# ACCtools/alignasm

Hardware: AMD Instinct MI355X
Metric: contigs_per_sec (higher is better)
Workload: dtype int64

## Files before the change

### alignasm_amd/csrc/aasm_gpu.hip

```cpp
#include <hip/hip_runtime.h>
#include <initializer_list>

#include <atomic>
#include <chrono>
#include <mutex>
#include <thread>
#include <fcntl.h>
#include <sys/mman.h>
#include <sys/stat.h>
#include <unistd.h>

#include "aasm_pipeline.h"
#include "aasm_ksw.h"
#include "aasm_cut.h"
#include "aasm_read.h"
#include "aasm_paf.hpp"

namespace aasm {

__device__ inline int64_t xcd_bid(int64_t b, int64_t g, int on) {
    if (!on || g < 64) return b;
    const int64_t g8 = g & ~(int64_t)7;
    return b < g8 ? (b & 7) * (g8 >> 3) + (b >> 3) : b;
}
// ... 177 lines not shown
        int64_t oa = sh_carry[0], ob = sh_carry[1], ta = 0, tb = 0;
#pragma unroll
        for (int i = 0; i < 16; i++) { const int64_t xa = sh_w[0][i], xb = sh_w[1][i]; if (i < wv) { oa += xa; ob += xb; } ta += xa; tb += xb; }
        int64_t ra = oa + ia - sa, rb = ob + ib - sb;
#pragma unroll
        for (int i = 0; i < 4; i++) { if (i0 + i < n) { out_a[i0 + i] = ra; if (in_b) out_b[i0 + i] = rb; } ra += va[i]; rb += vb[i]; }
        __syncthreads();
        if (threadIdx.x == 0) { sh_carry[0] += ta; sh_carry[1] += tb; }
        __syncthreads();
    }
    if (threadIdx.x == 0) { out_a[n] = sh_carry[0]; if (in_b) out_b[n] = sh_carry[1]; }
}

struct ScalarSrc { const int64_t *p[12]; };
__global__ void aasm_read_scalars(ScalarSrc src, int n, int64_t *dst) {
    const int i = (int)threadIdx.x;
    if (i < n) __hip_atomic_store(dst + i, *src.p[i], __ATOMIC_RELAXED, __HIP_MEMORY_SCOPE_SYSTEM);
}

struct ArenaBlock { char *p; size_t cap, used; };

struct DevCtx {
    int device = -1;
    bool ready = false;
    hipStream_t stream = nullptr, side = nullptr, side2 = nullptr;
    hipEvent_t ev_fork, ev_join, ev_fork2, ev_join2, ev_fork_b;
    int64_t *d_scratch2 = nullptr;
    size_t d_scratch2_cap = 0;
    std::vector<ArenaBlock> blocks;
    int64_t *pinned = nullptr;
    int64_t *pinned_dev = nullptr;
    char *stage[2] = {nullptr, nullptr};
    int64_t *d_scratch = nullptr;
    size_t d_scratch_cap = 0;
    uint64_t generation = 0;
    std::atomic<int> input_arrived{0};
    std::mutex mu;
    hipEvent_t ev_b[AASM_N_PHASES], ev_e[AASM_N_PHASES], ev_t0, ev_t1;
    int n_events_made = 0;
    int n_events2 = 0;
    hipEvent_t *timing_event(int i) { return i < AASM_N_PHASES ? &ev_b[i] : i < 2 * AASM_N_PHASES ? &ev_e[i - AASM_N_PHASES] : i == 2 * AASM_N_PHASES ? &ev_t0 : &ev_t1; }
    bool events = false;
    size_t peak_bytes = 0;
    std::vector<hipEvent_t> export_events;
};

static void drain_exports(DevCtx &cx) {
    for (hipEvent_t e : cx.export_events) { (void)hipEventSynchronize(e); (void)hipEventDestroy(e); }
    cx.export_events.clear();
}
static DevCtx g_ctx[16];
static std::mutex g_init_mu;
static std::atomic<int64_t> g_n_range_splits{0}, g_n_device_mallocs{0}, g_n_stream_syncs{0}, g_n_read_slow_rows{0}, g_n_read_fallbacks{0};

static std::string hip_err(const char *what, hipError_t e) {
    return std::string(what) + ": " + hipGetErrorString(e);
}

static int ctx_init(int device) {
    if (device < 0 || device >= 16) { set_last_error("device ordinal out of range"); return AASM_E_INVAL; }
    std::lock_guard<std::mutex> lk(g_init_mu);
    DevCtx &cx = g_ctx[device];
    if (cx.ready) return AASM_OK;
    int n = 0;
    hipError_t e = hipGetDeviceCount(&n);
    if (e != hipSuccess || n <= 0) { set_last_error("no HIP device available (this library has no CPU fallback)"); return AASM_E_NODEVICE; }
    if (device >= n) { set_last_error("device ordinal beyond hipGetDeviceCount"); return AASM_E_NODEVICE; }
    if ((e = hipSetDevice(device)) != hipSuccess) { set_last_error(hip_err("hipSetDevice", e)); return AASM_E_NODEVICE; }
    auto fail = [&](const char *what, hipError_t err) {
        set_last_error(hip_err(what, err));
        if (cx.pinned) { hipHostFree(cx.pinned); cx.pinned = nullptr; }
        if (cx.n_events_made > 0) { hipEventDestroy(cx.ev_fork); }
        if (cx.n_events_made > 1) { hipEventDestroy(cx.ev_join); }
        for (int i = 2; i < cx.n_events_made; i++) hipEventDestroy(*cx.timing_event(i - 2));
        cx.n_events_made = 0;
        if (cx.n_events2 > 0) { hipEventDestroy(cx.ev_fork2); }
        if (cx.n_events2 > 1) { hipEventDestroy(cx.ev_join2); }
        if (cx.n_events2 > 2) { hipEventDestroy(cx.ev_fork_b); }
        cx.n_events2 = 0;
        if (cx.side2) { hipStreamDestroy(cx.side2); cx.side2 = nullptr; }
        if (cx.side) { hipStreamDestroy(cx.side); cx.side = nullptr; }
        if (cx.stream) { hipStreamDestroy(cx.stream); cx.stream = nullptr; }
        return AASM_E_NODEVICE;
    };
    if ((e = hipStreamCreateWithFlags(&cx.stream, hipStreamNonBlocking)) != hipSuccess) return fail("hipStreamCreate", e);
    if ((e = hipStreamCreateWithFlags(&cx.side, hipStreamNonBlocking)) != hipSuccess) return fail("hipStreamCreate", e);
    if ((e = hipStreamCreateWithFlags(&cx.side2, hipStreamNonBlocking)) != hipSuccess) return fail("hipStreamCreate", e);
    if ((e = hipEventCreateWithFlags(&cx.ev_fork2, hipEventDisableTiming)) != hipSuccess) return fail("hipEventCreate", e);
    cx.n_events2 = 1;
    if ((e = hipEventCreateWithFlags(&cx.ev_join2, hipEventDisableTiming)) != hipSuccess) return fail("hipEventCreate", e);
    cx.n_events2 = 2;
    if ((e = hipEventCreateWithFlags(&cx.ev_fork_b, hipEventDisableTiming)) != hipSuccess) return fail("hipEventCreate", e);
    cx.n_events2 = 3;
    if ((e = hipEventCreateWithFlags(&cx.ev_fork, hipEventDisableTiming)) != hipSuccess) return fail("hipEventCreate", e);
    cx.n_events_made = 1;
    if ((e = hipEventCreateWithFlags(&cx.ev_join, hipEventDisableTiming)) != hipSuccess) return fail("hipEventCreate", e);
    cx.n_events_made = 2;
    for (int i = 0; i < 2 * AASM_N_PHASES + 2; i++) {
        if ((e = hipEventCreate(cx.timing_event(i))) != hipSuccess) return fail("hipEventCreate", e);
        cx.n_events_made++;
    }
    if ((e = hipHostMalloc((void **)&cx.pinned, 64 * sizeof(int64_t), hipHostMallocMapped)) != hipSuccess) return fail("hipHostMalloc", e);
    std::memset(cx.pinned, 0, 64 * sizeof(int64_t));
    if ((e = hipHostGetDevicePointer((void **)&cx.pinned_dev, cx.pinned, 0)) != hipSuccess) return fail("hipHostGetDevicePointer", e);
    cx.events = true;
    cx.device = device;
// ... 275 lines not shown

static thread_local int64_t g_bad_record = -1;

static int solve_on_device(DevCtx &cx, const aasm_batch_in &dev_in, const aasm_opts &opts, hipStream_t stream, aasm_result **res_out,
                           GpuBackend **be_out) {
    GpuBackend *be = *be_out;
    const bool timing = opts.collect_timing != 0;
    aasm_result *res = new aasm_result();
    res->device = cx.device; res->stream = stream;
    std::memset(&res->stats, 0, sizeof(res->stats));
    if (timing) hipEventRecord(cx.ev_t0, stream);
    be->test_dirty_scan = decode_hooks(opts).dirty_scan;
    int rc = run_pipeline(*be, dev_in, opts, res->w, res->sz);
    if (rc == AASM_OK) rc = pack_alloc(*be, res->w, res->pk);
    be->flush_zero();
    if (timing) hipEventRecord(cx.ev_t1, stream);
    be->join();
    be->join2();
    hipError_t e = hipStreamSynchronize(stream);
    if (e == hipSuccess) e = hipStreamSynchronize(cx.side);
    if (e == hipSuccess) e = hipStreamSynchronize(cx.side2);
    be->scan_stalled();
    if (rc == AASM_OK && be->failed()) rc = be->oom() ? AASM_E_NOMEM : AASM_E_HIP;
    if (rc == AASM_OK && e != hipSuccess) { set_last_error(hip_err("pipeline", e)); rc = AASM_E_HIP; }
    if (rc == AASM_E_PARSE) {
        g_bad_record = res->sz.bad_record;
        set_last_error("malformed cs:Z tag in record " + std::to_string(res->sz.bad_record) + " of the batch");
    }
    if (rc == AASM_E_HIP || rc == AASM_E_NOMEM || be->failed() || cx.pinned[SCAN_STALL_SLOT] != 0) {
        (void)hipDeviceSynchronize();
        if (cx.d_scratch) (void)hipMemset(cx.d_scratch, 0, cx.d_scratch_cap * 8);
        if (cx.d_scratch2) (void)hipMemset(cx.d_scratch2, 0, cx.d_scratch2_cap * 8);
        cx.pinned[SCAN_STALL_SLOT] = 0;
        (void)hipGetLastError();
    }
    if (rc != AASM_OK) { delete res; return rc; }
    if (timing) {
        for (int i = 0; i < AASM_N_PHASES; i++)
            if (be->phase_used[i]) { float ms = 0; if (hipEventElapsedTime(&ms, cx.ev_b[i], cx.ev_e[i]) == hipSuccess) res->stats.phase_ms[i] = ms; }
        float ms = 0;
        if (hipEventElapsedTime(&ms, cx.ev_t0, cx.ev_t1) == hipSuccess) res->stats.total_ms = ms;
    }
    {
        int64_t cnt[CNT_N];
        std::memset(cnt, 0, sizeof(cnt));
        be->d2h(cnt, res->w.counters, sizeof(cnt));
        aasm_stats &st = res->stats;
        st.n_vertices = res->sz.VT; st.n_edges = res->sz.ET;
        st.n_pairs = res->sz.S > 0 ? be->read_i64(res->w.ov_rank + res->sz.S) : 0;
        st.n_heap_nodes = cnt[CNT_HEAPNODES]; st.n_paths_found = cnt[CNT_PATHS]; st.n_paths_converted = cnt[CNT_CONVERTED];
        st.n_unconnectable = cnt[CNT_UNCONN]; st.range_steps = cnt[CNT_RANGE_STEPS];
        st.ispr_edges = cnt[CNT_ISPR_E]; st.ispr_vertices = cnt[CNT_ISPR_V]; st.path_edges = cnt[CNT_PATH_E];
        st.out_elems = cnt[CNT_OUT_E]; st.pq_pushes = cnt[CNT_PQ_PUSH];
        if (be->failed()) { delete res; return AASM_E_HIP; }
    }
    res->stats.device_bytes = (int64_t)be->bytes;
    res->generation = cx.generation;
    res->named = be->named;
    *res_out = res;
    return AASM_OK;
}

extern "C" {

int aasm_abi_version(void) { return AASM_ABI_VERSION; }

int aasm_device_count(void) {
    int n = 0;
    if (hipGetDeviceCount(&n) != hipSuccess) return 0;
    return n;
}

int aasm_init(int device) { return ctx_init(device); }

int aasm_solve_device(const aasm_batch_in *dev_in, const aasm_opts *opts, void *stream, aasm_result **res) {
    if (!dev_in || !res) return AASM_E_INVAL;
    aasm_opts o;
    std::memset(&o, 0, sizeof(o));
    if (opts) o = *opts;
    int rc = ctx_init(o.device);
    if (rc != AASM_OK) return rc;
    DevCtx &cx = g_ctx[o.device];
    std::lock_guard<std::mutex> lk(cx.mu);
    hipSetDevice(o.device);
    hipStream_t s = stream ? (hipStream_t)stream : cx.stream;
    GpuBackend be(cx, s, o.collect_timing != 0);
    GpuBackend *bp = &be;
    return solve_on_device(cx, *dev_in, o, s, res, &bp);
}

int aasm_result_stats(const aasm_result *res, aasm_stats *stats) {
    if (!res || !stats) return AASM_E_INVAL;
    *stats = res->stats;
    return AASM_OK;
}

namespace {
#define AASM_STAGE_BYTES ((size_t)16 << 20)
struct FetchBackend {
    DevCtx &cx; hipStream_t stream; bool fail = false;
    void d2h(void *dst, const void *src, size_t n) {
        if (fail || n == 0) return;
        hipError_t e = hipMemcpyAsync(dst, src, n, hipMemcpyDeviceToHost, stream);
        if (e == hipSuccess) e = hipStreamSynchronize(stream);
        if (e != hipSuccess) { set_last_error(hip_err("hipMemcpy D2H", e)); fail = true; }
    }
// ... 191 lines not shown
    std::vector<int32_t> ones((size_t)n_contigs, 1);
    w.dupflag = (int32_t *)m.up(ones.data(), (size_t)n_contigs * 4);
#if defined(AASM_KPROF)
    w.prof_heap = (int64_t *)filled((size_t)n_contigs * 64, 0);
#endif
    if (!m.ok) return be.err();
    launch_kernel(KN_SORT_FIX, n_contigs, kern_block[KN_SORT_FIX], be.stream, w);
    if (!be.launched() || !be.d2h(perm_out, w.perm, (size_t)R * 4)) return be.err();
#if defined(AASM_KPROF)
    {
        std::vector<int64_t> kp((size_t)n_contigs * 8);
        be.d2h(kp.data(), w.prof_heap, kp.size() * 8);
        double mean[8] = {0};
        for (int64_t c = 0; c < n_contigs; c++) for (int i = 0; i < 8; i++) mean[i] += (double)kp[(size_t)c * 8 + i] / (double)n_contigs;
        fprintf(stderr, "sort_fix sections (mean cycles): load %.0f  A %.0f  B %.0f  C %.0f  global partitions %.0f  wave lifetime %.1f us\n", mean[0], mean[1], mean[2], mean[3], mean[4], mean[7] / 100.0);
    }
#endif
    return AASM_OK;
}

int aasm_sssp_dijkstra(int64_t n_graphs, const int64_t *g_voff, const int64_t *rowptr, const int32_t *col, const int64_t *w5,
                       const int32_t *src, int64_t *d5, int32_t *prev, int device) {
    const char *why = "";
    const int rc = dijkstra_check_args(n_graphs, g_voff, rowptr, col, w5, src, d5, prev, &why);
    return graph_entry("aasm_sssp_dijkstra", rc, why, device, [&](GraphGpu &be) { return dijkstra_run(be, n_graphs, g_voff, rowptr, col, w5, src, d5, prev, &why); });
}

int aasm_sssp_dial(int64_t n_graphs, const int64_t *g_voff, const int64_t *rowptr, const int32_t *col, const int32_t *cost,
                   const int32_t *src, int lim, int64_t *dist, int64_t *pre, int device) {
    const char *why = "";
    const int rc = dial_check_args(n_graphs, g_voff, rowptr, col, cost, src, lim, dist, pre, &why);
    return graph_entry("aasm_sssp_dial", rc, why, device, [&](GraphGpu &be) { return dial_run(be, n_graphs, g_voff, rowptr, col, cost, src, lim, dist, pre, &why); });
}

int aasm_k_shortest_walks(int64_t n_graphs, const int64_t *g_voff, const int64_t *rowptr, const int32_t *col, const int64_t *w5,
                          const int32_t *source, const int32_t *sink, int64_t k, int flags, int device, aasm_ksw_out *out) {
    const char *why = "";
    const int rc = ksw_check_args(n_graphs, g_voff, rowptr, col, w5, source, sink, k, flags, out, &why);
    return graph_entry("aasm_k_shortest_walks", rc, why, device, [&](GraphGpu &be) {
        return ksw_run(be, n_graphs, g_voff, rowptr, col, w5, source, sink, k, flags, out, (int64_t)4 << 30);
    });
}

void aasm_ksw_free(aasm_ksw_out *out) { ksw_free_out(out); }

int64_t aasm_debug_counter(const char *name) {
    if (!name) return -1;
    const std::string n(name);
    if (n == "range_splits") return g_n_range_splits.load();
    if (n == "device_mallocs") return g_n_device_mallocs.load();
    if (n == "stream_syncs") return g_n_stream_syncs.load();
    if (n == "read_slow_rows") return g_n_read_slow_rows.load();
    if (n == "read_host_fallbacks") return g_n_read_fallbacks.load();
    return -1;
}

int64_t aasm_debug_fetch(aasm_result *res, const char *name, void *dst, int64_t dst_bytes) {
    if (!res || !name) return AASM_E_INVAL;
    DevCtx &cx = g_ctx[res->device];
    std::lock_guard<std::mutex> lk(cx.mu);
    if (res->generation != cx.generation) return AASM_E_INVAL;
    auto it = res->named.find(name);
    if (it == res->named.end()) return AASM_E_INVAL;
    if (dst) {
        hipSetDevice(res->device);
        size_t n = std::min<size_t>((size_t)dst_bytes, it->second.second);
        hipError_t e = hipMemcpy(dst, it->second.first, n, hipMemcpyDeviceToHost);
        if (e != hipSuccess) { set_last_error(hip_err("debug fetch", e)); return AASM_E_HIP; }
    }
    return (int64_t)it->second.second;
}

struct aasm_upload { int device; std::vector<void *> ptrs; aasm_batch_in view; };

static int upload_range(const aasm_batch_in *in, int64_t c0, int64_t c1, int device, aasm_upload **up_out, aasm_batch_in *dev_view) {
    if (!in || !up_out || !dev_view || c0 < 0 || c1 > in->n_contigs || c0 >= c1) return AASM_E_INVAL;
    int rc = ctx_init(device);
    if (rc != AASM_OK) return rc;
    hipSetDevice(device);
    g_ctx[device].input_arrived.store(1);
    aasm_upload *up = new aasm_upload();
    up->device = device;
    bool ok = true, oom = false;
    std::string why = "the batch carries neither match ranges nor cs tags";
    auto put = [&](const void *src, size_t bytes) -> void * {
        void *p = nullptr;
        if (!ok) return nullptr;
        hipError_t e = hipMalloc(&p, bytes ? bytes : 8);
        if (e != hipSuccess) { ok = false; oom = (e == hipErrorOutOfMemory); (void)hipGetLastError(); why = hip_err("hipMalloc(upload)", e); return nullptr; }
        up->ptrs.push_back(p);
        if (bytes && (e = hipMemcpy(p, src, bytes, hipMemcpyHostToDevice)) != hipSuccess) { ok = false; why = hip_err("hipMemcpy H2D", e); }
        return p;
    };
    const int64_t C = c1 - c0, r0 = in->ctg_rec_off[c0], r1 = in->ctg_rec_off[c1], R = r1 - r0;
    const int64_t g0 = in->rec_rng_off[r0], g1 = in->rec_rng_off[r1], G = g1 - g0;
    std::vector<int64_t> coff(C + 1), roff(R + 1);
    for (int64_t c = 0; c <= C; c++) coff[c] = in->ctg_rec_off[c0 + c] - r0;
    for (int64_t r = 0; r <= R; r++) roff[r] = in->rec_rng_off[r0 + r] - g0;
    aasm_batch_in &v = up->view;
    v.n_contigs = C; v.n_records = R; v.n_ranges = G;
    v.ctg_rec_off = (const int64_t *)put(coff.data(), (C + 1) * 8);
    v.qry_str = (const int64_t *)put(in->qry_str + r0, R * 8);
    v.qry_end = (const int64_t *)put(in->qry_end + r0, R * 8);
    v.ref_str = (const int64_t *)put(in->ref_str + r0, R * 8);
    v.ref_end = (const int64_t *)put(in->ref_end + r0, R * 8);
    v.qry_total = (const int64_t *)put(in->qry_total + r0, R * 8);
// ... 406 lines not shown
```

### alignasm_amd/csrc/aasm_kernels.h

```cpp
#pragma once
#include <cstddef>
#include "aasm_dev.h"
#include "../../include/alignasm_amd.h"

namespace aasm {

struct PqK;
struct WS {
    int64_t C, R, R0, S, VT, ET;
    int32_t K, nsl;
    int32_t avg_sidetracks;
    int32_t xcd_map;
    int32_t mw_compact;
    int32_t sort_depth_test;
    const int64_t *rec_off, *in_qs, *in_qe, *in_rs, *in_re, *in_qt, *in_rng_off, *rql, *rqr, *rrl;
    const int32_t *in_chr;
    const uint8_t *in_fwd, *in_mq;
    const char *cs_text;
    const int64_t *cs_off;
    int64_t *rng_rec;
    int64_t rng_stride;
    int32_t *cs_bad;
    int32_t *perm, *dupflag, *np, *pstart;
    int64_t *s_qs, *s_qe, *s_rs, *s_re, *s_qt, *s_rb;
// ... 24 lines not shown
    I4 *kcand;
    PqK *pq;
    int64_t pq_stride;
    int32_t *pathA, *pathB, *pathT, *pre2, *stamp;
    Dist *dist2;
    uint8_t *notalt;
    int32_t *mark_time;
    int32_t *plan_kk;
    int32_t *nconv, *cv_ctg, *cv_k, *cv_ord, *cv_kind, *cv_szr, *cv_szv, *cv_n, *cv_err, *cv_path, *cv_pre2, *cv_stamp, *cv_la;
    int64_t *conv_off, *cv_roff, *cv_voff, *cv_cov;
    OutElem *cv_out;
    Dist *cv_dist2;
    int64_t NCONV;
    OutElem *cur_out, *main_out, *alt_out, *pool;
    int32_t *main_len, *alt_len, *all_gen, *all_seq;
    int32_t *ar_ctg, *ar_gen, *ar_seq, *ar_len;
    int64_t *ar_off;
    int64_t pool_cap, ar_cap;
    int64_t *main_off, *alt_off;
    OutElem *main_c, *alt_c;
    int32_t *status;
    int64_t *counters;
    int32_t *gb_flag; int32_t gb_off;
    int64_t *prof_heap, *prof_sel, *prof_gb;
    Dist *st_cost;
    int32_t *st_n;
    I4 *vhdr, *vhdr2, *cinfo;
    int32_t mw_mode;
    int32_t *mw_flag, *mw_lg;
    HNode *hprov;
    int64_t *mw_off;
    int32_t *mw_cap;
    int32_t *mw_order, *mw_rs, *mw_fb;
    int32_t *mw_rsv, *mw_used;
    int32_t *mw_list, *mw_sorted;
    int32_t *mw_key;
    int32_t mw_n, mw_base;
    I4 *tnx;
    int32_t *tnx16;
    I4 *rvh;
    I4 *r_pk;
    I4 *fvh;
    int32_t chain_mode;
    int32_t chain_all, chain_minN;
    int32_t chain_test;
    int32_t *chain_flag, *chain_list;
    int32_t *pend;
    int32_t *cq;
    I4 *bfsq;
    int32_t chain_ord;
    int32_t chain_rn;
};

enum { CNT_RANGE_STEPS = 0, CNT_UNCONN, CNT_POOL, CNT_AR, CNT_CONVERTED, CNT_HEAPNODES, CNT_PATHS, CNT_OVF, CNT_ISPR_E, CNT_ISPR_V, CNT_PATH_E, CNT_OUT_E, CNT_PQ_PUSH, CNT_MW, CNT_MAXN, CNT_LONGSORT, CNT_MAXV, CNT_CHAIN, CNT_GB_S, CNT_GB_L, CNT_GB_REST, CNT_N };

AASM_DEV void set_status(const WS &w, int64_t c, int code) { if (w.status[c] == 0) w.status[c] = code; }
AASM_DEV bool in_chain_class(const WS &w, int64_t c) { return w.chain_flag != nullptr && w.chain_flag[c] != 0; }
AASM_DEV bool in_graph_class(const WS &w, int64_t c) { return w.gb_flag && w.gb_flag[c] != 0; }
#define AASM_COORD_LIMIT ((int64_t)1 << 40)
AASM_DEV bool coord_ok(int64_t x) { return x >= 0 && x < AASM_COORD_LIMIT; }

struct CsScan {
    int64_t q, rr, val, n, cnt, o0;
    int32_t plen;
    int t;
    bool fwd, bad;
};
AASM_DEV void cs_close_op(CsScan &s, const WS &w) {
    if (s.t == ':') {
        if (s.plen < 1 || s.val <= 0 || s.n >= s.cnt) { s.bad = true; return; }
        if (s.fwd) {
            const int64_t o = s.o0 + s.n;
            I4 lo, hi; const int64_t qr = s.q + s.val - 1;
            lo.x = lo32((uint64_t)s.q); lo.y = hi32((uint64_t)s.q); lo.z = lo32((uint64_t)qr); lo.w = hi32((uint64_t)qr);
            hi.x = lo32((uint64_t)s.rr); hi.y = hi32((uint64_t)s.rr); hi.z = 0; hi.w = 0;
            I4 *rec = (I4 *)(w.rng_rec + 4 * o); rec[0] = lo; rec[1] = hi;
            s.q += s.val;
        } else {
            const int64_t o = s.o0 + s.cnt - 1 - s.n;
            I4 lo, hi; const int64_t ql = s.q - s.val, qr = s.q - 1, rl = s.rr + s.val - 1;
            lo.x = lo32((uint64_t)ql); lo.y = hi32((uint64_t)ql); lo.z = lo32((uint64_t)qr); lo.w = hi32((uint64_t)qr);
            hi.x = lo32((uint64_t)rl); hi.y = hi32((uint64_t)rl); hi.z = 0; hi.w = 0;
            I4 *rec = (I4 *)(w.rng_rec + 4 * o); rec[0] = lo; rec[1] = hi;
            s.q -= s.val;
        }
        s.rr += s.val;
        s.n++;
    } else if (s.t == '*') {
        if (s.plen != 2) { s.bad = true; return; }
        s.q += s.fwd ? 1 : -1; s.rr += 1;
    } else {
        if (s.plen < 1) { s.bad = true; return; }
        if (s.t == '+') s.q += s.fwd ? s.plen : -s.plen; else s.rr += s.plen;
    }
}
AASM_DEV void kb_cs_ranges(const KCtx &k, const WS &w) {
    const int64_t br = k.bid * k.nthreads + k.tid;
    if (br >= w.R) return;
    const int64_t r = w.R0 + br;
    const int64_t p0 = w.cs_off[r], len = w.cs_off[r + 1] - p0;
    const uint8_t *cs = (const uint8_t *)w.cs_text + p0;
    const int64_t qs = w.in_qs[r], qe = w.in_qe[r], rs = w.in_rs[r], re = w.in_re[r];
    CsScan s;
    s.fwd = w.in_fwd[r] != 0;
    s.o0 = w.in_rng_off[r]; s.cnt = w.in_rng_off[r + 1] - s.o0;
    s.q = s.fwd ? qs : qe + 1; s.rr = s.fwd ? rs : re;
    s.val = 0; s.n = 0; s.plen = 0; s.t = 0;
// ... 1367 lines not shown
        for (int i = 0; i < GB_U; i++) {
            const int64_t e = eb + (en[i] & 0xffffu);
            const bool in = p0 + i * nth < E;
            hv[i] = in ? w.e_col[e] : 0; wq[i] = in ? w.e_wq[e] : 0; wr[i] = in ? w.e_wr[e] : 0; fl[i] = in ? w.e_fl[e] : 0;
        }
        AASM_UNROLL
        for (int i = 0; i < GB_U; i++) {
            if (p0 + i * nth >= E) break;
            const uint32_t key = en[i] & 0xffffu;
            const I4 rec = pack_in_edge((int32_t)(en[i] >> 16), wq[i], wr[i], fl[i]);
            const int32_t l0 = L->rp[hv[i]], l1 = L->rp[hv[i] + 1];
            int32_t rank = 0, j = l0;
            for (; j + 4 <= l1; j += 4) {
                const uint32_t k0 = L->ks[j], k1 = L->ks[j + 1], k2 = L->ks[j + 2], k3 = L->ks[j + 3];
                rank += (k0 < key) + (k1 < key) + (k2 < key) + (k3 < key);
            }
            for (; j < l1; j++) rank += (L->ks[j] < key) ? 1 : 0;
            w.r_pk[eb + l0 + rank] = rec;
            if (rank < 2) w.rvh[3 * (vb + hv[i]) + 1 + rank] = rec;
        }
    }
    KPROF_STAMP(3);
    for (int32_t v0 = tid; v0 < V; v0 += GB_U * nth) {
        int64_t o0[GB_U], o1[GB_U];
        I4 f1[GB_U];
        AASM_UNROLL
        for (int i = 0; i < GB_U; i++) { const int32_t v = v0 + i * nth; const bool in = v < V; o0[i] = in ? w.rowptr[vb + v] : 0; o1[i] = in ? w.rowptr[vb + v + 1] : 0; }
        AASM_UNROLL
        for (int i = 0; i < GB_U; i++) f1[i] = fwd_hdr_heads(w, o0[i], o1[i]);
        AASM_UNROLL
        for (int i = 0; i < GB_U; i++) {
            const int32_t v = v0 + i * nth;
            if (v >= V) break;
            const int64_t gv = vb + v;
            const int32_t ideg = L->rp[v + 1] - L->rp[v];
            const int64_t r0 = eb + L->rp[v];
            I4 h, z;
            z.x = z.y = z.z = z.w = 0;
            h.x = (int32_t)(uint32_t)(uint64_t)r0; h.y = (int32_t)((uint64_t)r0 >> 32); h.z = ideg; h.w = 0;
            w.rptr[gv] = r0;
            w.rvh[3 * gv] = h;
            if (ideg < 1) w.rvh[3 * gv + 1] = z;
            if (ideg < 2) w.rvh[3 * gv + 2] = z;
            sweep_vertex_store(w, gv, ideg, o0[i], o1[i], f1[i], vb + V);
        }
    }
    KPROF_STAMP(4);
    KPROF_FLUSH(w.prof_gb, c, tid);
}

#ifndef AASM_SWEEP_G
#define AASM_SWEEP_G (AASM_WAVE >= 32 ? 32 : 1)
#endif
template <int G> struct SweepGrp {
    static constexpr int N = AASM_WAVE / G;
    int g, gl;
    AASM_MEM explicit SweepGrp(int lane) : g(lane / G), gl(lane % G) {}
    AASM_MEM uint32_t bits(uint64_t m) const { return G >= 64 ? 0u : (uint32_t)((m >> (g * (G & 63))) & ((1ull << (G & 63)) - 1ull)); }
    AASM_MEM int32_t below(uint64_t m) const {
        if (G >= 64) return popc64(m & lanemask_lt(gl));
        return __builtin_popcount(bits(m) & ((1u << gl) - 1u));
    }
    AASM_MEM int32_t count(uint64_t m) const { return G >= 64 ? popc64(m) : __builtin_popcount(bits(m)); }
};

struct ChainSync { int32_t tail_pub, sweep_done, prep_done, ord_pub, ord_done, pad[3]; };
#if defined(AASM_HOST_EMUL)
AASM_DEV void st_shared_i32(int32_t *p, int32_t v) { *p = v; }
#else
AASM_DEV void st_shared_i32(int32_t *p, int32_t v) { __hip_atomic_store(p, v, __ATOMIC_RELAXED, __HIP_MEMORY_SCOPE_WORKGROUP); }
#endif

template <int G, bool PUB = false>
AASM_DEV void kb_rev_sweep(const KCtx &k, const WS &w, ChainSync *S = nullptr) {
    const SweepGrp<G> sg(k.lane);
    const int64_t c = k.bid * SweepGrp<G>::N + sg.g;
    const bool valid = c < w.C && (PUB || !in_chain_class(w, c));
    const int64_t V = valid ? (int64_t)w.ctgV[c] : 0;
    const int64_t vb = valid ? w.voff[c] : 0;
    RevQ *Q = (RevQ *)k.lds + sg.g;
    Dist *d = w.sp_d + vb;
    int32_t *best = w.sp_best + vb, *q = w.rev_order + vb, *cnt = w.cnt_tmp + vb;
    const I4 *rvh = w.rvh + 3 * vb;
    int32_t tail = 0, lds_hi = 0;
    for (int64_t base = 0; wave_any(base < V); base += G) {
        const int64_t v = base + sg.gl;
        const bool z = v < V && cnt[v] == 0;
        const uint64_t m = wave_ballot(z);
        const int32_t at = tail + sg.below(m);
        if (z) {
            q[at] = (int32_t)v;
            if (at < REVQ_N) { RevEnt *E = &Q->e[at]; I4 hd = rvh[3 * v]; hd.w = (int32_t)v; E->hdr = hd; E->d = d[v]; E->rec[0] = rvh[3 * v + 1]; E->rec[1] = rvh[3 * v + 2]; }
        }
        tail += sg.count(m);
    }
    lds_hi = tail < REVQ_N ? tail : REVQ_N;
    wave_lds_sync();
    int32_t pub = 0;
    if (PUB) { pub = uni(tail); store_drain(); st_shared_i32(&S->tail_pub, pub); }
    int32_t head = 0;
    while (wave_any(head < tail)) {
        const bool live = head < tail;
        RevEnt *E = &Q->e[head & (REVQ_N - 1)];
        if (wave_any(live && head >= lds_hi)) {
            if (live && head >= lds_hi && sg.gl == 0) { const int32_t v = q[head]; I4 hd = rvh[3 * v]; hd.w = v; E->hdr = hd; E->d = d[v]; E->rec[0] = rvh[3 * v + 1]; E->rec[1] = rvh[3 * v + 2]; }
            wave_lds_sync();
        }
        I4 hd; hd.x = hd.y = hd.z = hd.w = 0;
        Dist dv = dist_max();
        if (live) { hd = E->hdr; dv = E->d; head++; }
        const int32_t deg = hd.z, v = hd.w;
        const int64_t r0 = (int64_t)(((uint64_t)(uint32_t)hd.y << 32) | (uint32_t)hd.x);
        const bool reach = dv.anom >= 0;
        for (int32_t base = 0; wave_any(base < deg); base += G) {
            const int32_t t = base + sg.gl;
            const bool act = t < deg;
            bool z = false;
            int32_t u = 0;
            I4 uh0, uh1, uh2;
            Dist du = dist_max();
            uh0.x = uh0.y = uh0.z = uh0.w = 0; uh1 = uh0; uh2 = uh0;
            if (act) {
                I4 rc;
                if (t < 2) rc = E->rec[t];
                else { rc = w.r_pk[r0 + t]; asm volatile("" ::: "memory"); }
                u = rc.x;
                Dist wd;
                wd.qry = (int64_t)(((uint64_t)(uint32_t)rc.z << 32) | (uint32_t)rc.y); wd.ref = rc.w & 0xffffff;
                const int32_t fl = (int32_t)((uint32_t)rc.w >> 24);
                wd.anom = fl & 3; wd.qnz = (fl >> 2) & 1; wd.qtot = (fl >> 3) & 1; wd.pad = 0;
                du = d[u];
                const int32_t left = cnt[u] - 1;
                uh0 = rvh[3 * u]; uh1 = rvh[3 * u + 1]; uh2 = rvh[3 * u + 2];
                const Dist cand = dist_add(dv, wd);
                const int64_t sc = cand.qry + cand.ref, su = du.qry + du.ref;
                const int32_t tc = cand.qtot ? cand.qtot : 1, tu = du.qtot ? du.qtot : 1;
                const bool better = reach & ((du.anom < 0) | (sc < su) | ((sc == su) & ((cand.anom < du.anom) | ((cand.anom == du.anom) & ((int64_t)cand.qnz * tu > (int64_t)du.qnz * tc)))));
                if (better) { du = cand; d[u] = cand; best[u] = v; }
                cnt[u] = left;
                z = left == 0;
            }
            const uint64_t m = wave_ballot(z);
            const int32_t at = tail + sg.below(m);
            if (z) {
                q[at] = u;
                if (lds_hi == tail && at - head < REVQ_N - 1) { RevEnt *N = &Q->e[at & (REVQ_N - 1)]; uh0.w = u; N->hdr = uh0; N->d = du; N->rec[0] = uh1; N->rec[1] = uh2; }
            }
            const int32_t nnew = sg.count(m);
            if (lds_hi == tail) { int32_t room = REVQ_N - 1 - (tail - head); if (room > nnew) room = nnew; if (room < 0) room = 0; lds_hi += room; }
            tail += nnew;
        }
        wave_lds_sync();
        if (PUB) {
            const int32_t tu = uni(tail);
            if (tu != pub) { store_drain(); st_shared_i32(&S->tail_pub, tu); pub = tu; }
        }
    }
    if (valid && tail != (int32_t)V && sg.gl == 0) set_status(w, c, -6);
    if (PUB) { store_drain(); st_shared_i32(&S->sweep_done, 1); }
}

struct FwdEnt { I4 a, b; };
struct FwdQ { FwdEnt e[REVQ_N]; };
#define AASM_FWD_LDS_BYTES (REVQ_N * 32)
static_assert(sizeof(FwdQ) <= AASM_FWD_LDS_BYTES, "LDS budget");
template <int G>
AASM_DEV void kb_fwd_sweep(const KCtx &k, const WS &w) {
    const SweepGrp<G> sg(k.lane);
    const int64_t c = k.bid * SweepGrp<G>::N + sg.g;
    const bool valid = c < w.C;
    const int64_t V = valid ? (int64_t)w.ctgV[c] : 0;
    const int64_t vb = valid ? w.voff[c] : 0;
    FwdQ *Q = (FwdQ *)k.lds + sg.g;
    int32_t *q = w.fwd_order + vb, *pos = w.fwd_pos + vb, *cnt = w.cnt_tmp2 + vb, *an = w.an + vb;
    const I4 *fvh = w.fvh + 2 * vb;
    int32_t tail = 0, lds_hi = 0;
    for (int64_t base = 0; wave_any(base < V); base += G) {
        const int64_t v = base + sg.gl;
        const bool z = v < V && cnt[v] == 0;
        const uint64_t m = wave_ballot(z);
        if (z) {
            const int32_t t = tail + sg.below(m);
            q[t] = (int32_t)v; pos[v] = t;
            if (t < REVQ_N) { I4 fa = fvh[2 * v], fb = fvh[2 * v + 1]; fa.w = (int32_t)v; fb.x = an[v]; Q->e[t].a = fa; Q->e[t].b = fb; }
        }
        tail += sg.count(m);
    }
    lds_hi = tail < REVQ_N ? tail : REVQ_N;
    wave_lds_sync();
    int32_t head = 0;
    while (wave_any(head < tail)) {
        const bool live = head < tail;
        FwdEnt *E = &Q->e[head & (REVQ_N - 1)];
        if (wave_any(live && head >= lds_hi)) {
            if (live && head >= lds_hi && sg.gl == 0) { const int32_t u = q[head]; I4 fa = fvh[2 * u], fb = fvh[2 * u + 1]; fa.w = u; fb.x = an[u]; E->a = fa; E->b = fb; }
            wave_lds_sync();
        }
        I4 fa, fb; fa.x = fa.y = fa.z = fa.w = 0; fb = fa;
        if (live) { fa = E->a; fb = E->b; head++; }
        const int32_t deg = fa.z, au = fb.x;
        const int64_t r0 = (int64_t)(((uint64_t)(uint32_t)fa.y << 32) | (uint32_t)fa.x);
        for (int32_t base = 0; wave_any(base < deg); base += G) {
            const int32_t t = base + sg.gl;
            const bool act = t < deg;
            bool z = false;
            int32_t v = 0, av = -1;
            I4 va, vbb;
            va.x = va.y = va.z = va.w = 0; vbb = va;
            if (act) {
                int32_t wa;
                if (t < 2) { v = t == 0 ? fb.y : fb.z; wa = (fb.w >> (8 * t)) & 3; }
                else { v = w.e_col[r0 + t]; wa = w.e_fl[r0 + t] & 3; }
                av = an[v];
                const int32_t left = cnt[v] - 1;
                va = fvh[2 * v]; vbb = fvh[2 * v + 1];
                const int32_t nd = au + wa;
                if ((au >= 0) & ((av < 0) | (nd < av))) { av = nd; an[v] = nd; }
                cnt[v] = left;
                z = left == 0;
            }
            const uint64_t m = wave_ballot(z);
            const int32_t at = tail + sg.below(m);
            if (z) {
                q[at] = v; pos[v] = at;
                if (lds_hi == tail && at - head < REVQ_N - 1) { FwdEnt *N = &Q->e[at & (REVQ_N - 1)]; va.w = v; vbb.x = av; N->a = va; N->b = vbb; }
            }
            const int32_t nnew = sg.count(m);
            if (lds_hi == tail) { int32_t room = REVQ_N - 1 - (tail - head); if (room > nnew) room = nnew; if (room < 0) room = 0; lds_hi += room; }
            tail += nnew;
        }
        wave_lds_sync();
    }
    if (valid && sg.gl == 0 && V > 0) {
        w.anom_dest[c] = an[V - 1];
        if (tail != (int32_t)V) set_status(w, c, -6);
    }
}

AASM_DEV void kb_topo_count(const KCtx &k, const WS &w) {
    const int64_t gp = k.bid * k.nthreads + k.tid;
    if (gp >= w.VT) return;
    const int64_t vb = w.voff[w.v_ctg[gp]];
    const int32_t u = w.fwd_order[gp];
    w.tp_deg[gp] = (int32_t)(w.rowptr[vb + u + 1] - w.rowptr[vb + u]);
    w.tp_vj[gp] = w.v_j[vb + u];
}
AASM_DEV void kb_topo_fill(const KCtx &k, const WS &w) {
    const int64_t gp = k.bid * AASM_WAVE + k.lane;
    const bool act = gp < w.VT;
    int64_t vb = 0, r0 = 0, t0 = 0;
    int32_t deg = 0;
    if (act) {
        vb = w.voff[w.v_ctg[gp]];
        const int32_t u = w.fwd_order[gp];
        r0 = w.rowptr[vb + u]; deg = w.tp_deg[gp]; t0 = w.tp_ptr[gp];
    }
    const bool big = deg > AASM_LONG_ROW;
    if (act && !big)
        for (int32_t t = 0; t < deg; t++) {
            w.te_pk[t0 + t] = pack_in_edge(w.fwd_pos[vb + w.e_col[r0 + t]], w.e_wq[r0 + t], w.e_wr[r0 + t], w.e_fl[r0 + t]);
        }
    uint64_t bigmask = wave_ballot(big);
    while (bigmask) {
        const int src = ffs64(bigmask) - 1;
        bigmask &= bigmask - 1;
        const int64_t vb2 = wave_bcast(vb, src), r02 = wave_bcast(r0, src), t02 = wave_bcast(t0, src);
        const int32_t deg2 = wave_bcast(deg, src);
        for (int32_t t = k.lane; t < deg2; t += AASM_WAVE) {
            w.te_pk[t02 + t] = pack_in_edge(w.fwd_pos[vb2 + w.e_col[r02 + t]], w.e_wq[r02 + t], w.e_wr[r02 + t], w.e_fl[r02 + t]);
        }
    }
}

AASM_DEV int32_t children_vertex(const WS &w, int64_t gv, int32_t *ch4 = nullptr) {
    const int64_t vb = w.voff[w.v_ctg[gv]];
    const int32_t u = (int32_t)(gv - vb);
    const int64_t r0 = w.rptr[gv], r1 = w.rptr[gv + 1];
    int32_t n = 0, prev = -1;
    int32_t c0 = -1, c1 = -1, c2 = -1, c3 = -1;
    for (int64_t t = r0; t < r1; t += 4) {
        int32_t src[4], bst[4];
        AASM_UNROLL
        for (int i = 0; i < 4; i++) src[i] = (t + i < r1) ? w.r_pk[t + i].x : -1;
        AASM_UNROLL
        for (int i = 0; i < 4; i++) bst[i] = src[i] >= 0 ? w.sp_best[vb + src[i]] : -1;
// ... 2302 lines not shown
```

Baseline: 445,800.

## Process two queue vertices per iteration in reverse and forward topo sweeps

Both the reverse and the forward topological sweep kernels now consume two queued vertices per loop iteration when one has low degree. Their edges are packed into the same subgroup lanes, which cuts the number of serial wave iterations and LDS syncs on chain-like graphs. Conflicts where the second vertex depends on the first are found with ballots: the reverse sweep falls back to a single vertex, and the forward sweep folds the dependent update into one lane. New counters track how many pairs are formed. This adds branch complexity and register pressure, and any error in the dependency handling could change the results.

```diff
diff --git a/alignasm_amd/csrc/aasm_gpu.hip b/alignasm_amd/csrc/aasm_gpu.hip
--- a/alignasm_amd/csrc/aasm_gpu.hip
+++ b/alignasm_amd/csrc/aasm_gpu.hip
@@ -253,6 +253,7 @@
 static DevCtx g_ctx[16];
 static std::mutex g_init_mu;
 static std::atomic<int64_t> g_n_range_splits{0}, g_n_device_mallocs{0}, g_n_stream_syncs{0}, g_n_read_slow_rows{0}, g_n_read_fallbacks{0};
+static std::atomic<int64_t> g_n_sweep_pairs_rev{0}, g_n_sweep_pairs_fwd{0};
 
 static std::string hip_err(const char *what, hipError_t e) {
     return std::string(what) + ": " + hipGetErrorString(e);
@@ -634,6 +635,7 @@
         st.n_unconnectable = cnt[CNT_UNCONN]; st.range_steps = cnt[CNT_RANGE_STEPS];
         st.ispr_edges = cnt[CNT_ISPR_E]; st.ispr_vertices = cnt[CNT_ISPR_V]; st.path_edges = cnt[CNT_PATH_E];
         st.out_elems = cnt[CNT_OUT_E]; st.pq_pushes = cnt[CNT_PQ_PUSH];
+        g_n_sweep_pairs_rev += cnt[CNT_PAIR_REV]; g_n_sweep_pairs_fwd += cnt[CNT_PAIR_FWD];
         if (be->failed()) { delete res; return AASM_E_HIP; }
     }
     res->stats.device_bytes = (int64_t)be->bytes;
@@ -931,6 +933,8 @@
     if (n == "stream_syncs") return g_n_stream_syncs.load();
     if (n == "read_slow_rows") return g_n_read_slow_rows.load();
     if (n == "read_host_fallbacks") return g_n_read_fallbacks.load();
+    if (n == "sweep_pairs_rev") return g_n_sweep_pairs_rev.load();
+    if (n == "sweep_pairs_fwd") return g_n_sweep_pairs_fwd.load();
     return -1;
 }
 
diff --git a/alignasm_amd/csrc/aasm_kernels.h b/alignasm_amd/csrc/aasm_kernels.h
--- a/alignasm_amd/csrc/aasm_kernels.h
+++ b/alignasm_amd/csrc/aasm_kernels.h
@@ -100,7 +100,7 @@
     int32_t chain_rn;
 };
 
-enum { CNT_RANGE_STEPS = 0, CNT_UNCONN, CNT_POOL, CNT_AR, CNT_CONVERTED, CNT_HEAPNODES, CNT_PATHS, CNT_OVF, CNT_ISPR_E, CNT_ISPR_V, CNT_PATH_E, CNT_OUT_E, CNT_PQ_PUSH, CNT_MW, CNT_MAXN, CNT_LONGSORT, CNT_MAXV, CNT_CHAIN, CNT_GB_S, CNT_GB_L, CNT_GB_REST, CNT_N };
+enum { CNT_RANGE_STEPS = 0, CNT_UNCONN, CNT_POOL, CNT_AR, CNT_CONVERTED, CNT_HEAPNODES, CNT_PATHS, CNT_OVF, CNT_ISPR_E, CNT_ISPR_V, CNT_PATH_E, CNT_OUT_E, CNT_PQ_PUSH, CNT_MW, CNT_MAXN, CNT_LONGSORT, CNT_MAXV, CNT_CHAIN, CNT_GB_S, CNT_GB_L, CNT_GB_REST, CNT_PAIR_REV, CNT_PAIR_FWD, CNT_N };
 
 AASM_DEV void set_status(const WS &w, int64_t c, int code) { if (w.status[c] == 0) w.status[c] = code; }
 AASM_DEV bool in_chain_class(const WS &w, int64_t c) { return w.chain_flag != nullptr && w.chain_flag[c] != 0; }
@@ -1574,6 +1574,15 @@
 #ifndef AASM_SWEEP_G
 #define AASM_SWEEP_G (AASM_WAVE >= 32 ? 32 : 1)
 #endif
+#ifndef AASM_SWEEP_PAIR
+#define AASM_SWEEP_PAIR 1
+#endif
+#ifndef AASM_SWEEP_PAIR_REV
+#define AASM_SWEEP_PAIR_REV AASM_SWEEP_PAIR
+#endif
+#ifndef AASM_SWEEP_PAIR_FWD
+#define AASM_SWEEP_PAIR_FWD AASM_SWEEP_PAIR
+#endif
 template <int G> struct SweepGrp {
     static constexpr int N = AASM_WAVE / G;
     int g, gl;
@@ -1584,6 +1593,7 @@
         return __builtin_popcount(bits(m) & ((1u << gl) - 1u));
     }
     AASM_MEM int32_t count(uint64_t m) const { return G >= 64 ? popc64(m) : __builtin_popcount(bits(m)); }
+    AASM_MEM bool any(uint64_t m) const { return G >= 64 ? m != 0 : bits(m) != 0u; }
 };
 
 struct ChainSync { int32_t tail_pub, sweep_done, prep_done, ord_pub, ord_done, pad[3]; };
@@ -1620,7 +1630,8 @@
     wave_lds_sync();
     int32_t pub = 0;
     if (PUB) { pub = uni(tail); store_drain(); st_shared_i32(&S->tail_pub, pub); }
-    int32_t head = 0;
+    constexpr bool PAIR = AASM_SWEEP_PAIR_REV != 0 && G > 1;
+    int32_t head = 0, npair = 0;
     while (wave_any(head < tail)) {
         const bool live = head < tail;
         RevEnt *E = &Q->e[head & (REVQ_N - 1)];
@@ -1628,6 +1639,69 @@
             if (live && head >= lds_hi && sg.gl == 0) { const int32_t v = q[head]; I4 hd = rvh[3 * v]; hd.w = v; E->hdr = hd; E->d = d[v]; E->rec[0] = rvh[3 * v + 1]; E->rec[1] = rvh[3 * v + 2]; }
             wave_lds_sync();
         }
+        if constexpr (PAIR) {
+        RevEnt *E1 = &Q->e[(head + 1) & (REVQ_N - 1)];
+        bool pair = live && head + 1 < lds_hi;
+        int32_t deg0 = 0, deg1 = 0;
+        if (live) deg0 = E->hdr.z;
+        if (pair) deg1 = E1->hdr.z;
+        pair = pair && (deg0 <= 2 || deg1 <= 2);
+        if (!pair) deg1 = 0;
+        for (int32_t base = 0; wave_any(base < deg0 + deg1); base += G) {
+            const int32_t t = base + sg.gl;
+            const bool e1 = t >= deg0;
+            const int32_t te = e1 ? t - deg0 : t;
+            bool act = t < deg0 + deg1;
+            const RevEnt *Em = e1 ? E1 : E, *Eo = e1 ? E : E1;
+            bool z = false;
+            int32_t u = 0, v = 0, left = 0;
+            I4 uh0, uh1, uh2, rc;
+            Dist du = dist_max(), dv = dist_max();
+            uh0.x = uh0.y = uh0.z = uh0.w = 0; uh1 = uh0; uh2 = uh0; rc = uh0;
+            if (act) {
+                const I4 hd = Em->hdr;
+                dv = Em->d; v = hd.w;
+                const int64_t r0 = (int64_t)(((uint64_t)(uint32_t)hd.y << 32) | (uint32_t)hd.x);
+                if (te < 2) rc = Em->rec[te];
+                else { rc = w.r_pk[r0 + te]; asm volatile("" ::: "memory"); }
+                u = rc.x;
+                du = d[u];
+                left = cnt[u] - 1;
+                uh0 = rvh[3 * u]; uh1 = rvh[3 * u + 1]; uh2 = rvh[3 * u + 2];
+            }
+            if (wave_any(pair && base <= deg0)) {
+                const int32_t od = e1 ? deg0 : deg1;
+                bool cf = false;
+                if (act && pair && base <= deg0 && od <= 2) cf = (od > 0 && u == Eo->rec[0].x) || (od > 1 && u == Eo->rec[1].x);
+                if (sg.any(wave_ballot(cf))) { pair = false; deg1 = 0; act = act && !e1; }
+            }
+            if (act) {
+                Dist wd;
+                wd.qry = (int64_t)(((uint64_t)(uint32_t)rc.z << 32) | (uint32_t)rc.y); wd.ref = rc.w & 0xffffff;
+                const int32_t fl = (int32_t)((uint32_t)rc.w >> 24);
+                wd.anom = fl & 3; wd.qnz = (fl >> 2) & 1; wd.qtot = (fl >> 3) & 1; wd.pad = 0;
+                const bool reach = dv.anom >= 0;
+                const Dist cand = dist_add(dv, wd);
+                const int64_t sc = cand.qry + cand.ref, su = du.qry + du.ref;
+                const int32_t tc = cand.qtot ? cand.qtot : 1, tu = du.qtot ? du.qtot : 1;
+                const bool better = reach & ((du.anom < 0) | (sc < su) | ((sc == su) & ((cand.anom < du.anom) | ((cand.anom == du.anom) & ((int64_t)cand.qnz * tu > (int64_t)du.qnz * tc)))));
+                if (better) { du = cand; d[u] = cand; best[u] = v; }
+                cnt[u] = left;
+                z = left == 0;
+            }
+            const uint64_t m = wave_ballot(z);
+            const int32_t at = tail + sg.below(m);
+            if (z) {
+                q[at] = u;
+                if (lds_hi == tail && at - head < REVQ_N) { RevEnt *N = &Q->e[at & (REVQ_N - 1)]; uh0.w = u; N->hdr = uh0; N->d = du; N->rec[0] = uh1; N->rec[1] = uh2; }
+            }
+            const int32_t nnew = sg.count(m);
+            if (lds_hi == tail) { int32_t room = REVQ_N - (tail - head); if (room > nnew) room = nnew; if (room < 0) room = 0; lds_hi += room; }
+            tail += nnew;
+        }
+        if (live) head += pair ? 2 : 1;
+        npair += pair ? 1 : 0;
+        } else {
         I4 hd; hd.x = hd.y = hd.z = hd.w = 0;
         Dist dv = dist_max();
         if (live) { hd = E->hdr; dv = E->d; head++; }
@@ -1672,6 +1746,7 @@
             if (lds_hi == tail) { int32_t room = REVQ_N - 1 - (tail - head); if (room > nnew) room = nnew; if (room < 0) room = 0; lds_hi += room; }
             tail += nnew;
         }
+        }
         wave_lds_sync();
         if (PUB) {
             const int32_t tu = uni(tail);
@@ -1679,6 +1754,7 @@
         }
     }
     if (valid && tail != (int32_t)V && sg.gl == 0) set_status(w, c, -6);
+    if (PAIR && npair > 0 && sg.gl == 0) atomic_add(&w.counters[CNT_PAIR_REV], (int64_t)npair);
     if (PUB) { store_drain(); st_shared_i32(&S->sweep_done, 1); }
 }
 
@@ -1710,7 +1786,8 @@
     }
     lds_hi = tail < REVQ_N ? tail : REVQ_N;
     wave_lds_sync();
-    int32_t head = 0;
+    constexpr bool PAIR = AASM_SWEEP_PAIR_FWD != 0 && G > 1;
+    int32_t head = 0, npair = 0;
     while (wave_any(head < tail)) {
         const bool live = head < tail;
         FwdEnt *E = &Q->e[head & (REVQ_N - 1)];
@@ -1719,6 +1796,67 @@
             wave_lds_sync();
         }
         I4 fa, fb; fa.x = fa.y = fa.z = fa.w = 0; fb = fa;
+        if constexpr (PAIR) {
+        const FwdEnt *E1 = &Q->e[(head + 1) & (REVQ_N - 1)];
+        I4 ga, gb; ga = fa; gb = fa;
+        bool pair = live && head + 1 < lds_hi;
+        if (live) { fa = E->a; fb = E->b; }
+        if (pair) { ga = E1->a; gb = E1->b; }
+        const int32_t deg0 = fa.z;
+        pair = pair && deg0 <= 2;
+        const int32_t deg1 = pair ? ga.z : 0;
+        const uint64_t pm = wave_ballot(pair);
+        for (int32_t base = 0; wave_any(base < deg0 + deg1); base += G) {
+            const int32_t t = base + sg.gl;
+            const bool e1 = t >= deg0;
+            const int32_t te = e1 ? t - deg0 : t;
+            const bool act = t < deg0 + deg1;
+            const I4 ma = e1 ? ga : fa, mb = e1 ? gb : fb;
+            const int32_t au = mb.x;
+            const int64_t r0 = (int64_t)(((uint64_t)(uint32_t)ma.y << 32) | (uint32_t)ma.x);
+            bool z = false;
+            int32_t v = 0, av = -1, wa = 0, left = 0, k = -1;
+            I4 va, vbb;
+            va.x = va.y = va.z = va.w = 0; vbb = va;
+            if (act) {
+                if (te < 2) { v = te == 0 ? mb.y : mb.z; wa = (mb.w >> (8 * te)) & 3; }
+                else { v = w.e_col[r0 + te]; wa = w.e_fl[r0 + te] & 3; }
+                av = an[v];
+                left = cnt[v] - 1;
+                va = fvh[2 * v]; vbb = fvh[2 * v + 1];
+                if (pair && e1 && base == 0) k = (deg0 > 0 && v == fb.y) ? 0 : (deg0 > 1 && v == fb.z) ? 1 : -1;
+            }
+            bool sup = false;
+            if (base == 0 && pm != 0) {
+                const uint64_t m0 = wave_ballot(k == 0), m1 = wave_ballot(k == 1);
+                sup = pair && !e1 && sg.any(t == 0 ? m0 : m1);
+            }
+            if (act && !sup) {
+                bool dirty = false;
+                if (k >= 0) {
+                    const int32_t nd0 = fb.x + ((fb.w >> (8 * k)) & 3);
+                    if ((fb.x >= 0) & ((av < 0) | (nd0 < av))) { av = nd0; dirty = true; }
+                    left -= 1;
+                }
+                const int32_t nd = au + wa;
+                if ((au >= 0) & ((av < 0) | (nd < av))) { av = nd; dirty = true; }
+                if (dirty) an[v] = av;
+                cnt[v] = left;
+                z = left == 0;
+            }
+            const uint64_t m = wave_ballot(z);
+            const int32_t at = tail + sg.below(m);
+            if (z) {
+                q[at] = v; pos[v] = at;
+                if (lds_hi == tail && at - head < REVQ_N) { FwdEnt *N = &Q->e[at & (REVQ_N - 1)]; va.w = v; vbb.x = av; N->a = va; N->b = vbb; }
+            }
+            const int32_t nnew = sg.count(m);
+            if (lds_hi == tail) { int32_t room = REVQ_N - (tail - head); if (room > nnew) room = nnew; if (room < 0) room = 0; lds_hi += room; }
+            tail += nnew;
+        }
+        if (live) head += pair ? 2 : 1;
+        npair += pair ? 1 : 0;
+        } else {
         if (live) { fa = E->a; fb = E->b; head++; }
         const int32_t deg = fa.z, au = fb.x;
         const int64_t r0 = (int64_t)(((uint64_t)(uint32_t)fa.y << 32) | (uint32_t)fa.x);
@@ -1751,8 +1889,10 @@
             if (lds_hi == tail) { int32_t room = REVQ_N - 1 - (tail - head); if (room > nnew) room = nnew; if (room < 0) room = 0; lds_hi += room; }
             tail += nnew;
         }
+        }
         wave_lds_sync();
     }
+    if (PAIR && npair > 0 && sg.gl == 0) atomic_add(&w.counters[CNT_PAIR_FWD], (int64_t)npair);
     if (valid && sg.gl == 0 && V > 0) {
         w.anom_dest[c] = an[V - 1];
         if (tail != (int32_t)V) set_status(w, c, -6);
```

Result: no change. 448,800 (median of 6 runs) (+0.7%).
